# achinastone/Tensorium

Measured on AMD Instinct MI355X. Metric: fp32 SGEMM GFLOP/s (M=N=K=4096) + YOLOv3 conv-fwd images/s, higher is better.
Workload: dtype fp32; 1 GPU; sgemm_nn_4096x4096x4096; M=4096, N=4096, K=4096, parallelism=1 independent replicas, one process per GPU, no data-path collective

## Files before the change

tensorium_amd/csrc/conv1x1.hip:

```cpp
#include <algorithm>
#include <type_traits>

#include "tns_act.hpp"
#include "tns_internal.hpp"

namespace tns {
namespace {

typedef float floatx4 __attribute__((ext_vector_type(4)));

__device__ __forceinline__ void c1_dma16(const float* sbase, unsigned voff, unsigned lds) {
  unsigned keep;
  asm volatile(
      "s_mov_b32 %0, m0\n\ts_mov_b32 m0, %3\n\ts_nop 0\n\t"
      "global_load_lds_dwordx4 %1, %2\n\ts_mov_b32 m0, %0"
      : "=&s"(keep)
      : "v"(voff), "s"(sbase), "s"(lds)
      : "memory");
}

struct C1Args {
  const float* A;
  const float* X;
  float* C;
  const float* bias;
  int M, N, K, P, tiles_m, act;
  bool fuse;
  bool add;
};

template <int BM_, int BK_, int WM_, int WN_>
struct C1G {
  static constexpr int BM = BM_, BK = BK_, WM = WM_, WN = WN_;
  static constexpr int BN = 64 * WN, NW = WM * WN, NT = 64 * NW, NG = BK / 16;
  static constexpr int A_TILE = BK * BM, B_TILE = BK * BN, STAGE = A_TILE + B_TILE;
  static constexpr int AU = BM * BK / 4 / NT;
  static constexpr int RPI = 256 / BN;
  static constexpr int BDMA = BK / RPI;
  static constexpr int DPW = (BDMA + NW - 1) / NW;
  static_assert(BM == 16 * WM && BK % 16 == 0 && 256 % BN == 0 && BK % RPI == 0, "geometry");
  static_assert(AU >= 1 && BM * BK / 4 % NT == 0, "A units");
  static_assert(2 * STAGE * 4 <= 65536, "LDS: several blocks per CU");
  static_assert(NG % 2 == 0, "groups: f0 holds group 0 at every tile start");
};

template <int N>
__device__ __forceinline__ void c1_wait(bool keep_n) {
  if (keep_n)
    asm volatile("s_waitcnt vmcnt(%0)" ::"n"(N) : "memory");
  else
    asm volatile("s_waitcnt vmcnt(0)" ::: "memory");
}

template <class G>
__global__ __launch_bounds__(G::NT) void conv1x1_kernel(C1Args p) {
  constexpr int BM = G::BM, BN = G::BN, BK = G::BK, NG = G::NG;
  constexpr int A_TILE = G::A_TILE, STAGE = G::STAGE, AU = G::AU, DPW = G::DPW;
  __shared__ __attribute__((aligned(16))) float smem[2 * STAGE];
  const int tid = threadIdx.x, lane = tid & 63;
  const int w = __builtin_amdgcn_readfirstlane(tid >> 6), wm = w % G::WM, wn = w / G::WM;
  const int r16 = lane & 15, q = lane >> 4;
  int tm, tn;
  {
    const int nb = gridDim.x, bid = blockIdx.x;
    const int xcd = bid & 7, qq = nb >> 3, rr = nb & 7;
    const int wg = (xcd < rr ? xcd * (qq + 1) : rr * (qq + 1) + (xcd - rr) * qq) + (bid >> 3);
    tm = wg % p.tiles_m;
    tn = wg / p.tiles_m;
  }
  const int m0 = tm * BM, n0 = tn * BN;
  const int N = p.N, K = p.K, P = p.P, nt = K / BK;
  const unsigned lds0 = (unsigned)(uintptr_t)(__attribute__((address_space(3))) float*)smem;
  unsigned b_off;
  {
    int n = n0 + 4 * (lane % (BN / 4));
    if (n > N - 4) n = N - 4;
    const int img = n / P, pix = n - img * P;
    b_off = 4u * (unsigned)(img * K * P + (lane / (BN / 4)) * P + pix);
  }
  auto dma_b = [&](int t, int st, int v) {
    int u = w + G::NW * v;
    if (G::BDMA % G::NW != 0 && u >= G::BDMA) u -= G::NW;
    c1_dma16(p.X + (int64_t)(t * BK + u * G::RPI) * P, b_off,
             lds0 + 4u * (unsigned)(st * STAGE + A_TILE) + 1024u * (unsigned)u);
  };
  auto dma_all = [&](int t, int st) {
#pragma unroll
    for (int v = 0; v < DPW; ++v) dma_b(t, st, v);
  };
  unsigned a_off[AU];
  int a_dst[AU];
#pragma unroll
  for (int u = 0; u < AU; ++u) {
    const int idx = tid + G::NT * u;
    const int lo = idx & 7, rest = idx >> 3;
    const int m = rest % BM, kq4 = lo + 8 * (rest / BM);
    const int mr = m0 + m < p.M ? m : p.M - 1 - m0;
    a_off[u] = 4u * (unsigned)(mr * K + 4 * kq4);
    a_dst[u] = (4 * (kq4 >> 2)) * BM * 4 + m * 4 + (kq4 & 3);
  }
  const float* a_row0 = p.A + (int64_t)m0 * K;
  floatx4 ra[AU];
  auto load_a = [&](int t) {
    const float* sb = a_row0 + t * BK;
#pragma unroll
    for (int u = 0; u < AU; ++u)
      asm volatile("global_load_dwordx4 %0, %1, %2" : "=v"(ra[u]) : "v"(a_off[u]), "s"(sb) : "memory");
  };
  auto store_a = [&](int st) {
    float* as = smem + st * STAGE;
#pragma unroll
    for (int u = 0; u < AU; ++u) {
      asm volatile("" : "+v"(ra[u]));
      as[a_dst[u]] = ra[u][0];
      as[a_dst[u] + BM * 4] = ra[u][1];
      as[a_dst[u] + 2 * BM * 4] = ra[u][2];
      as[a_dst[u] + 3 * BM * 4] = ra[u][3];
    }
  };

  floatx4 acc[4];
#pragma unroll
  for (int j = 0; j < 4; ++j) acc[j] = floatx4{0.f, 0.f, 0.f, 0.f};
  struct Frag {
    floatx4 a, b[4];
  };
  auto frag = [&](int st, int g, Frag& f) {
    const float* ap = smem + st * STAGE + ((4 * g + q) * BM + wm * 16 + r16) * 4;
    f.a = *reinterpret_cast<const floatx4*>(ap);
    const float* bp = smem + st * STAGE + A_TILE + (16 * g + q) * BN + wn * 64 + 4 * r16;
#pragma unroll
    for (int i = 0; i < 4; ++i) f.b[i] = *reinterpret_cast<const floatx4*>(bp + 4 * i * BN);
  };
  auto mma = [&](const Frag& f) {
#pragma unroll
    for (int i = 0; i < 4; ++i)
#pragma unroll
      for (int j = 0; j < 4; ++j)
        acc[j] = __builtin_amdgcn_mfma_f32_16x16x4f32(f.a[i], f.b[i][j], acc[j], 0, 0, 0);
  };
  auto mma_dma = [&](const Frag& f, int tb, int st) {
    constexpr int NM = 16, STEP = NM / DPW > 0 ? NM / DPW : 1;
#pragma unroll
    for (int x = 0; x < NM; ++x) {
      const int i = x / 4, j = x % 4;
      acc[j] = __builtin_amdgcn_mfma_f32_16x16x4f32(f.a[i], f.b[i][j], acc[j], 0, 0, 0);
      if (x % STEP == 0 && x / STEP < DPW) dma_b(tb, st, x / STEP);
      __builtin_amdgcn_sched_barrier(0);
    }
    if constexpr (NM / STEP < DPW) {
#pragma unroll
      for (int v = NM / STEP; v < DPW; ++v) dma_b(tb, st, v);
    }
  };

  Frag f0, f1;
  load_a(0);
  dma_all(0, 0);
  c1_wait<0>(false);
  store_a(0);
  if (nt > 1) {
    load_a(1);
    dma_all(1, 1);
  }
  __syncthreads();
  frag(0, 0, f0);
  for (int t = 0; t < nt; ++t) {
    const int cur = t & 1, nxt = cur ^ 1;
#pragma unroll
    for (int g = 0; g + 1 < NG; ++g) {
      Frag& fc = (g & 1) ? f1 : f0;
      Frag& fn = (g & 1) ? f0 : f1;
      frag(cur, g + 1, fn);
      __builtin_amdgcn_sched_barrier(0);
      mma(fc);
      __builtin_amdgcn_sched_barrier(0);
    }
    Frag& fl = f1;
    Frag& ff = f0;
    if (t + 1 < nt) {
      c1_wait<0>(false);
      store_a(nxt);
      __syncthreads();
      frag(nxt, 0, ff);
      if (t + 2 < nt) {
        load_a(t + 2);
        __builtin_amdgcn_sched_barrier(0);
        mma_dma(fl, t + 2, cur);
      } else {
        __builtin_amdgcn_sched_barrier(0);
        mma(fl);
      }
    } else {
      mma(fl);
    }
  }

  const int n = n0 + wn * 64 + 4 * r16;
  if (n >= N) return;
  const int img = n / P, pix = n - img * P;
#pragma unroll
  for (int e = 0; e < 4; ++e) {
    const int m = m0 + wm * 16 + 4 * q + e;
    if (m >= p.M) continue;
    const float bi = p.fuse ? p.bias[m] : 0.0f;
    floatx4 v = {acc[0][e], acc[1][e], acc[2][e], acc[3][e]};
    if (p.fuse) {
#pragma unroll
      for (int j = 0; j < 4; ++j) v[j] = act_apply_cheap(v[j] + bi, p.act);
    }
    floatx4* cp = reinterpret_cast<floatx4*>(p.C + ((int64_t)img * p.M + m) * P + pix);
    if (p.add) {
      const floatx4 o = *cp;
#pragma unroll
      for (int j = 0; j < 4; ++j) v[j] = o[j] + v[j];
    }
    *cp = v;
  }
}

struct C1Form {
  int bm, bn, bk;
  hipError_t (*fn)(const C1Args&, hipStream_t);
  const char* name;
};

template <class G>
hipError_t launch_c1(const C1Args& a, hipStream_t s) {
  const int64_t blocks = (int64_t)a.tiles_m * ((a.N + G::BN - 1) / G::BN);
  hipLaunchKernelGGL((conv1x1_kernel<G>), dim3((unsigned)blocks), dim3(G::NT), 0, s, a);
  return hipGetLastError();
}

#define TNS_C1(BMv, BKv, WMv, WNv) \
  {BMv, 64 * WNv, BKv, launch_c1<C1G<BMv, BKv, WMv, WNv>>, "conv1x1<" #BMv "x" #WNv "x64x" #BKv ">"}
const C1Form kC1[] = {
    TNS_C1(32, 32, 2, 1),
    TNS_C1(64, 32, 4, 1),
    TNS_C1(32, 64, 2, 1),
    TNS_C1(32, 32, 2, 2),
    TNS_C1(16, 32, 1, 2),
};
#undef TNS_C1
constexpr int kNumC1 = sizeof(kC1) / sizeof(kC1[0]);

}

int conv1x1_count() { return kNumC1; }
const char* conv1x1_name(int v) { return v >= 0 && v < kNumC1 ? kC1[v].name : ""; }

int conv1x1_pick(int64_t M, int64_t N, int64_t K, int64_t P) {
  (void)M; (void)N;
  if (P % 4 || P < 2704 || K % 32) return -1;
  return 3;
}

__global__ __launch_bounds__(256) void c1_transpose_kernel(const float* __restrict__ in,
                                                           float* __restrict__ out, int rows,
                                                           int cols) {
  __shared__ float t[32][33];
  const int c0 = blockIdx.x * 32, r0 = blockIdx.y * 32;
  const int tx = threadIdx.x & 31, ty = threadIdx.x >> 5;
  for (int y = ty; y < 32; y += 8) {
    const int r = r0 + y, c = c0 + tx;
    t[y][tx] = r < rows && c < cols ? in[(int64_t)r * cols + c] : 0.0f;
  }
  __syncthreads();
  for (int y = ty; y < 32; y += 8) {
    const int c = c0 + y, r = r0 + tx;
    if (c < cols && r < rows) out[(int64_t)c * rows + r] = t[tx][y];
  }
}

hipError_t launch_transpose(const float* in, float* out, int64_t rows, int64_t cols,
                            hipStream_t s) {
  if (rows <= 0 || cols <= 0) return hipSuccess;
  if (rows > (1 << 26) || cols > (1 << 26)) return hipErrorInvalidValue;
  hipLaunchKernelGGL(c1_transpose_kernel,
                     dim3((unsigned)((cols + 31) / 32), (unsigned)((rows + 31) / 32)), dim3(256), 0,
                     s, in, out, (int)rows, (int)cols);
  return hipGetLastError();
}

hipError_t launch_conv1x1(int v, const float* weights, const float* x, const float* bias,
                          float* out, int64_t batch, int64_t M, int64_t K, int64_t P, int act,
                          hipStream_t s, bool add) {
  if (v < 0 || v >= kNumC1) return hipErrorInvalidValue;
  const C1Form& f = kC1[v];
  const int64_t N = batch * P;
  if (P % 4 || K % f.bk || M < 1 || N < 4 || batch * K * P * 4 > 0x7fffffffLL ||
      M * K * 4 > 0x7fffffffLL || (reinterpret_cast<uintptr_t>(weights) & 15) ||
      (reinterpret_cast<uintptr_t>(x) & 15) || (reinterpret_cast<uintptr_t>(out) & 15))
    return hipErrorInvalidValue;
  C1Args a{};
  a.A = weights; a.X = x; a.C = out; a.bias = bias;
  a.M = (int)M; a.N = (int)N; a.K = (int)K; a.P = (int)P;
  a.tiles_m = (int)((M + f.bm - 1) / f.bm); a.act = act; a.fuse = bias != nullptr; a.add = add;
  if ((int64_t)a.tiles_m * ((N + f.bn - 1) / f.bn) > 0x7fffffffLL) return hipErrorInvalidValue;
  return f.fn(a, s);
}

}
```

tensorium_amd/csrc/conv_slab.hip:

```cpp
#include <algorithm>
#include <type_traits>

#include "tns_act.hpp"
#include "tns_internal.hpp"

namespace tns {
namespace {

typedef float floatx4 __attribute__((ext_vector_type(4)));

__device__ __forceinline__ void slab_dma16(const float* sbase, unsigned voff, unsigned lds) {
  unsigned keep;
  asm volatile(
      "s_mov_b32 %0, m0\n\ts_mov_b32 m0, %3\n\ts_nop 0\n\t"
      "global_load_lds_dwordx4 %1, %2\n\ts_mov_b32 m0, %0"
      : "=&s"(keep)
      : "v"(voff), "s"(sbase), "s"(lds)
      : "memory");
}

struct SlabFillArgs {
  const float* x;
  int64_t strideX;
  float* slab;
  int C, H, W, stride, pad, dil, ow, ohw, N, K, KT;
  float inv_ohw, inv_ow;
  unsigned bytes;
  int64_t units;
};

__device__ __forceinline__ int slab_div(int n, int d, float inv) {
  int qq = (int)((float)n * inv);
  while (qq * d > n) --qq;
  while ((qq + 1) * d <= n) ++qq;
  return qq;
}

template <int KS, int BK, int BN>
__global__ __launch_bounds__(256) void slab_fill_kernel(SlabFillArgs a) {
  constexpr int NG = BK / 16, KK = KS * KS;
  const int64_t x = (int64_t)blockIdx.x * 256 + threadIdx.x;
  if (x >= a.units) return;
  const int c = (int)(x % BN);
  const int64_t r1 = x / BN;
  const int g = (int)(r1 % NG);
  const int64_t r2 = r1 / NG;
  const int t = (int)(r2 % a.KT), ct = (int)(r2 / a.KT);
  const int n = ct * BN + c;
  float v[16];
  const __amdgpu_buffer_rsrc_t rsrc =
      __builtin_amdgcn_make_buffer_rsrc(const_cast<float*>(a.x), 0, a.bytes, 0x00020000);
  {
    const int nn = n < a.N ? n : a.N - 1;
    const int img = slab_div(nn, a.ohw, a.inv_ohw), pix = nn - img * a.ohw;
    const int oy = slab_div(pix, a.ow, a.inv_ow), ox = pix - oy * a.ow;
    const int iy0 = oy * a.stride - a.pad, ix0 = ox * a.stride - a.pad;
    const int HW = a.H * a.W;
    unsigned mask = 0;
    int toff[KK];
#pragma unroll
    for (int kr = 0; kr < KS; ++kr)
#pragma unroll
      for (int kc = 0; kc < KS; ++kc) {
        const int iy = iy0 + kr * a.dil, ix = ix0 + kc * a.dil;
        mask |= (unsigned)(((unsigned)iy < (unsigned)a.H) & ((unsigned)ix < (unsigned)a.W))
                << (kr * KS + kc);
        toff[kr * KS + kc] = 4 * (kr * a.dil * a.W + kc * a.dil);
      }
    if (n >= a.N) mask = 0;
    const unsigned base = 4u * (unsigned)(img * (int)a.strideX + iy0 * a.W + ix0);
    const int k0 = t * BK + 16 * g;
    int ch = k0 / KK, tap = k0 - ch * KK;
#pragma unroll
    for (int e = 0; e < 16; ++e) {
      int off = toff[0];
#pragma unroll
      for (int u = 1; u < KK; ++u) off = tap == u ? toff[u] : off;
      const unsigned o = ((mask >> tap) & 1u) ? base + 4u * (unsigned)(ch * HW) + (unsigned)off
                                              : 0x80000000u;
      v[e] = __builtin_bit_cast(float, __builtin_amdgcn_raw_buffer_load_b32(rsrc, o, 0, 0));
      if (++tap == KK) {
        tap = 0;
        ++ch;
      }
    }
  }
  float* dst = a.slab + ((r2 * NG + g) * 4 * BN + c) * 4;
#pragma unroll
  for (int q = 0; q < 4; ++q)
    *reinterpret_cast<floatx4*>(dst + q * BN * 4) = floatx4{v[q], v[4 + q], v[8 + q], v[12 + q]};
}

template <int KS, int BK, int BN>
__global__ __launch_bounds__((BN + 63) / 64 * 64) void slab_fill_u_kernel(SlabFillArgs a) {
  constexpr int NG = BK / 16, KK = KS * KS;
  const int c = threadIdx.x;
  if (c >= BN) return;
  const int64_t r1 = blockIdx.x;
  const int g = (int)(r1 % NG);
  const int64_t r2 = r1 / NG;
  const int t = (int)(r2 % a.KT), ct = (int)(r2 / a.KT);
  const int n = ct * BN + c;
  float v[16];
  const __amdgpu_buffer_rsrc_t rsrc =
      __builtin_amdgcn_make_buffer_rsrc(const_cast<float*>(a.x), 0, a.bytes, 0x00020000);
  {
    const int nn = n < a.N ? n : a.N - 1;
    const int img = slab_div(nn, a.ohw, a.inv_ohw), pix = nn - img * a.ohw;
    const int oy = slab_div(pix, a.ow, a.inv_ow), ox = pix - oy * a.ow;
    const int iy0 = oy * a.stride - a.pad, ix0 = ox * a.stride - a.pad;
    const int HW = a.H * a.W;
    unsigned mask = 0;
#pragma unroll
    for (int kr = 0; kr < KS; ++kr)
#pragma unroll
      for (int kc = 0; kc < KS; ++kc) {
        const int iy = iy0 + kr * a.dil, ix = ix0 + kc * a.dil;
        mask |= (unsigned)(((unsigned)iy < (unsigned)a.H) & ((unsigned)ix < (unsigned)a.W))
                << (kr * KS + kc);
      }
    if (n >= a.N) mask = 0;
    const unsigned base = 4u * (unsigned)(img * (int)a.strideX + iy0 * a.W + ix0);
    const int k0 = __builtin_amdgcn_readfirstlane(t * BK + 16 * g);
    int ch = k0 / KK, tap = k0 - ch * KK;
    int kr = tap / KS, kc = tap - kr * KS;
#pragma unroll
    for (int e = 0; e < 16; ++e) {
      const unsigned uoff = 4u * (unsigned)(ch * HW + kr * a.dil * a.W + kc * a.dil);
      const unsigned o = ((mask >> tap) & 1u) ? base + uoff : 0x80000000u;
      v[e] = __builtin_bit_cast(float, __builtin_amdgcn_raw_buffer_load_b32(rsrc, o, 0, 0));
      ++tap;
      if (++kc == KS) {
        kc = 0;
        ++kr;
      }
      if (tap == KK) {
        tap = 0;
        kr = 0;
        ++ch;
      }
    }
  }
  float* dst = a.slab + ((r2 * NG + g) * 4 * BN + c) * 4;
#pragma unroll
  for (int q = 0; q < 4; ++q)
    *reinterpret_cast<floatx4*>(dst + q * BN * 4) = floatx4{v[q], v[4 + q], v[8 + q], v[12 + q]};
}

struct SlabGemmArgs {
  const float* A;
  const float* slab;
  float* C;
  const float* bias;
  int M, N, K, KT, tiles_m, ohw, act;
  bool fuse;
};

template <int BM_, int BN_, int BK_, int WM_, int WN_, int JA_, int NA_, int NS_, int DG_ = 0,
          int MAP_ = 0>
struct SG {
  static constexpr int BM = BM_, BN = BN_, BK = BK_, WM = WM_, WN = WN_, JA = JA_, NA = NA_;
  static constexpr int NS = NS_;
  static constexpr int DG = DG_, MAP = MAP_;
  static constexpr int NW = WM * WN, NT = 64 * NW, J = BN / 16, NG = BK / 16, ROWS = BK / 4;
  static constexpr int JB = NA < WN ? (J - NA * JA) / (WN - NA) : 0;
  static constexpr int A_TILE = ROWS * BM * 4, B_TILE = ROWS * BN * 4, STAGE = A_TILE + B_TILE;
  static constexpr int AU = BM * BK / 4 / NT;
  static constexpr int BDMA = 4 * BK * BN / 1024;
  static constexpr int DPW = (BDMA + NW - 1) / NW;
  static_assert(BM == 16 * WM && BN % 16 == 0 && BK % 16 == 0, "geometry");
  static_assert(NA * JA + (WN - NA) * JB == J && NA >= 1 && NA <= WN, "wave column split");
  static_assert(AU >= 1 && BM * BK / 4 % NT == 0, "A units");
  static_assert(4 * BK * BN % 1024 == 0, "whole DMA instructions");
  static_assert(NS >= 2 && NS * STAGE * 4 <= 163840, "LDS");
  static_assert(NG >= 2 && NG % 2 == 0, "groups: f0 holds group 0 at every tile start");
  static_assert(DPW * (NS - 2) <= 63 && DPW <= 63, "vmcnt immediates");
};

template <int JW>
struct SFrag {
  floatx4 a, b[JW];
};

template <int N>
__device__ __forceinline__ void wait_vm(bool keep_n) {
  if (keep_n)
    asm volatile("s_waitcnt vmcnt(%0)" ::"n"(N) : "memory");
  else
    asm volatile("s_waitcnt vmcnt(0)" ::: "memory");
}

template <class G>
__global__ __launch_bounds__(G::NT, 1) void slab_gemm_kernel(SlabGemmArgs p) {
  constexpr int BM = G::BM, BN = G::BN, BK = G::BK, NG = G::NG, NS = G::NS;
  constexpr int A_TILE = G::A_TILE, STAGE = G::STAGE, AU = G::AU, DPW = G::DPW;
  __shared__ __attribute__((aligned(16))) float smem[NS * STAGE];
  const int tid = threadIdx.x, lane = tid & 63;
  const int w = __builtin_amdgcn_readfirstlane(tid >> 6), wm = w % G::WM, wn = w / G::WM;
  const int r16 = lane & 15, q = lane >> 4;
  int tm, tn;
  {
    const int nb = gridDim.x, bid = blockIdx.x;
    const int xcd = bid & 7, qq = nb >> 3, rr = nb & 7;
    const int wg = (xcd < rr ? xcd * (qq + 1) : rr * (qq + 1) + (xcd - rr) * qq) + (bid >> 3);
    if constexpr (G::MAP == 1) {
      const int tiles_n = (p.N + BN - 1) / BN;
      tn = wg % tiles_n;
      tm = wg / tiles_n;
    } else {
      tm = wg % p.tiles_m;
      tn = wg / p.tiles_m;
    }
  }
  const int m0 = tm * BM, n0 = tn * BN;
  const int N = p.N, K = p.K, nt = p.KT;
  const float* slabT = p.slab + (int64_t)tn * K * BN;
  const unsigned lds0 = (unsigned)(uintptr_t)(__attribute__((address_space(3))) float*)smem;
  const unsigned voff = 16u * (unsigned)lane;
  auto dma_b = [&](int t, int st, int v) {
    if constexpr (G::DG & 1) return;
    int u = w + G::NW * v;
    if (G::BDMA % G::NW != 0 && u >= G::BDMA) u -= G::NW;
    slab_dma16(slabT + (int64_t)t * (BK * BN) + 256 * u, voff,
               lds0 + 4u * (unsigned)(st * STAGE + A_TILE) + 1024u * (unsigned)u);
  };
  auto dma_all = [&](int t, int st) {
#pragma unroll
    for (int v = 0; v < DPW; ++v) dma_b(t, st, v);
  };
  unsigned a_off[AU];
  int a_dst[AU];
#pragma unroll
  for (int u = 0; u < AU; ++u) {
    const int idx = tid + G::NT * u;
    const int lo = idx & 7, rest = idx >> 3;
    const int m = rest % BM, kq4 = lo + 8 * (rest / BM);
    a_off[u] = 4u * (unsigned)(m * K + 4 * kq4);
    a_dst[u] = (4 * (kq4 >> 2)) * BM * 4 + m * 4 + (kq4 & 3);
  }
  const float* a_row0 = p.A + (int64_t)m0 * K;
  floatx4 ra[AU];
  auto load_a = [&](int t) {
    if constexpr (G::DG & 2) return;
    const float* sb = a_row0 + t * BK;
#pragma unroll
    for (int u = 0; u < AU; ++u)
      asm volatile("global_load_dwordx4 %0, %1, %2" : "=v"(ra[u]) : "v"(a_off[u]), "s"(sb) : "memory");
  };
  auto store_a = [&](int st) {
    if constexpr (G::DG & 2) return;
    float* as = smem + st * STAGE;
#pragma unroll
    for (int u = 0; u < AU; ++u) {
      asm volatile("" : "+v"(ra[u]));
      as[a_dst[u]] = ra[u][0];
      as[a_dst[u] + BM * 4] = ra[u][1];
      as[a_dst[u] + 2 * BM * 4] = ra[u][2];
      as[a_dst[u] + 3 * BM * 4] = ra[u][3];
    }
  };

  auto run = [&](auto JWC, const int coff) {
    constexpr int JW = decltype(JWC)::value;
    floatx4 acc[JW];
#pragma unroll
    for (int j = 0; j < JW; ++j) acc[j] = floatx4{0.f, 0.f, 0.f, 0.f};
    using Frag = SFrag<JW>;
    auto frag = [&](int st, int g, Frag& f) {
      const float* ap = smem + st * STAGE + ((4 * g + q) * BM + wm * 16 + r16) * 4;
      f.a = *reinterpret_cast<const floatx4*>(ap);
      const float* bp = smem + st * STAGE + A_TILE + ((4 * g + q) * BN + coff * 16 + r16) * 4;
#pragma unroll
      for (int j = 0; j < JW; ++j) f.b[j] = *reinterpret_cast<const floatx4*>(bp + 64 * j);
    };
    auto mma = [&](const Frag& f) {
#pragma unroll
      for (int i = 0; i < 4; ++i)
#pragma unroll
        for (int j = 0; j < JW; ++j)
          acc[j] = __builtin_amdgcn_mfma_f32_16x16x4f32(f.a[i], f.b[j][i], acc[j], 0, 0, 0);
    };
    auto mma_dma = [&](const Frag& f, int tb, int st) {
      constexpr int NM = 4 * JW, STEP = NM / DPW > 0 ? NM / DPW : 1;
#pragma unroll
      for (int x = 0; x < NM; ++x) {
        const int i = x / JW, j = x % JW;
        acc[j] = __builtin_amdgcn_mfma_f32_16x16x4f32(f.a[i], f.b[j][i], acc[j], 0, 0, 0);
        if (x % STEP == 0 && x / STEP < DPW) dma_b(tb, st, x / STEP);
        __builtin_amdgcn_sched_barrier(0);
      }
      if constexpr (NM / STEP < DPW) {
#pragma unroll
        for (int v = NM / STEP; v < DPW; ++v) dma_b(tb, st, v);
      }
    };

    Frag f0, f1;
    load_a(0);
#pragma unroll
// ... 190 lines not shown
```

tensorium_amd/csrc/conv_tile4.hip:

```cpp
#include <type_traits>

#include "tns_act.hpp"
#include "tns_internal.hpp"

namespace tns {
namespace {

typedef float floatx4 __attribute__((ext_vector_type(4)));

template <int I, int N, class F>
__device__ __forceinline__ void cfor(F&& f) {
  if constexpr (I < N) {
    f(std::integral_constant<int, I>{});
    cfor<I + 1, N>(f);
  }
}

template <int JW>
struct Frag4 {
  floatx4 a, b[JW];
};

template <int BM_, int BN_, int WM_, int WN_, int BK_, int SG_, int IL_ = 0, bool SI_ = false,
          int RI_ = 0, bool ST_ = false, int JA_ = 0, int NA_ = 0, bool TA_ = false,
          bool DX_ = false, bool PF_ = false>
struct Geo4 {
  static constexpr bool PF = PF_;
  static constexpr bool DX = DX_;
  static constexpr bool TA = TA_;
  static constexpr int BM = BM_, BN = BN_, WM = WM_, WN = WN_, BK = BK_, SG = SG_;
  static constexpr int IL = IL_, RI = RI_;
  static constexpr bool SI = SI_, ST = ST_;
  static constexpr int NW = WM * WN, NT = 64 * NW;
  static constexpr int J = BN / 16;
  static constexpr int JA = JA_ > 0 ? JA_ : J / WN;
  static constexpr int NA = JA_ > 0 ? NA_ : WN;
  static constexpr int JB = NA < WN ? (J - NA * JA) / (WN - NA) : 0;
  static constexpr int NG = BK / 16;
  static constexpr int ROWS = BK / 4;
  static constexpr int A_TILE = ROWS * BM * 4;
  static constexpr int STAGE = ROWS * (BM + BN) * 4;
  static constexpr int AU = BM * BK / 4 / NT;
  static constexpr int KI = BK / 4 / NW;
  static_assert(BM == 16 * WM, "one 16-row strip per wave");
  static_assert(BM % 16 == 0 && BN % 16 == 0, "b128 slot rows: 64-dword multiples");
  static_assert(BK % 16 == 0 && SG <= NG - 2, "stores precede the barrier");
  static_assert(!(IL && SI) || SG >= 1 || PF_, "interleaved stores need a group after the loads");
  static_assert(!ST || (!IL && !SI && SG + 1 <= NG - 2 && NW % 2 == 0), "staggered staging");
  static_assert(AU >= 1 && BM * BK / 4 % NT == 0 && KI >= 1 && BK / 4 % NW == 0, "geometry");
  static_assert(NA * JA + (WN - NA) * JB == J && NA >= 1 && NA <= WN, "wave column split");
  static_assert(2 * STAGE * 4 + 64 <= 163840, "LDS");
  static_assert(!DX || TA, "DX: k-major weights");
  static_assert(!PF || !ST, "PF: register staging, no staggered halves");
  static constexpr int AST = 4 * AU;
  static constexpr int BLD = KI * J;
  static constexpr int BST = KI * J;
};

template <class G, int KS>
__global__ __launch_bounds__(G::NT) void conv_tile4_kernel(GemmArgs p, int dil) {
  constexpr int BM = G::BM, BN = G::BN, BK = G::BK, J = G::J, NG = G::NG;
  constexpr int A_TILE = G::A_TILE, STAGE = G::STAGE, AU = G::AU, KI = G::KI;
  __shared__ __attribute__((aligned(16))) float smem[2 * STAGE];
#ifdef TNS_CT4_STAMPS
  const unsigned long long rt_entry = __builtin_amdgcn_s_memrealtime();
#endif
  auto a_st = [&](int st) -> float* { return smem + st * STAGE; };
  auto b_st = [&](int st) -> float* { return smem + st * STAGE + A_TILE; };

  const int tid = threadIdx.x, lane = tid & 63, w = tid >> 6, wm = w % G::WM, wn = w / G::WM;
  const int half = __builtin_amdgcn_readfirstlane(w >= G::NW / 2 ? 1 : 0);
  const int r16 = lane & 15, q = lane >> 4;
  const int tiles_m = (int)(p.M / BM);
  int tm, tn;
  {
    const int nb = gridDim.x, bid = blockIdx.x;
    const int xcd = bid & 7, qq = nb >> 3, rr = nb & 7;
    const int wg = (xcd < rr ? xcd * (qq + 1) : rr * (qq + 1) + (xcd - rr) * qq) + (bid >> 3);
#if defined(TNS_CT4_MAP) && TNS_CT4_MAP == 1
    const int tiles_n = (int)((p.N + BN - 1) / BN);
    tn = wg % tiles_n;
    tm = wg / tiles_n;
#elif defined(TNS_CT4_MAP) && TNS_CT4_MAP == 2
    const int tiles_n = (int)((p.N + BN - 1) / BN);
    const int gm = min(4, tiles_m), per = gm * tiles_n, grp = wg / per;
    const int gs = min(gm, tiles_m - grp * gm), in = wg - grp * per;
    tm = grp * gm + in % gs;
    tn = in / gs;
#else
    tm = wg % tiles_m;
    tn = wg / tiles_m;
#endif
  }
  const int64_t m0 = (int64_t)tm * BM;
  const int n0 = tn * BN;
  const int N = (int)p.N, K = (int)p.K;
  const int H = p.conv_H, W = p.conv_W, HW = H * W;
  auto dx_pix = [&](int pix) -> int {
    if (!p.dx_cls) return pix;
    const int qy = pix / p.conv_ow, qx = pix - qy * p.conv_ow;
    return (2 * qy + ((p.dx_cls >> 1) & 1)) * p.dx_imgW + 2 * qx + ((p.dx_cls >> 2) & 1);
  };

  auto col_geo = [&](int n, unsigned& vb, unsigned& m) {
    n = n < N ? n : N - 1;
    const int img = n / p.conv_ohw, pix = n - img * p.conv_ohw;
    const int orow = pix / p.conv_ow, ocol = pix - orow * p.conv_ow;
    const int ir0 = orow * p.conv_sY - p.conv_pH, ic0 = ocol * p.conv_sX - p.conv_pW;
    vb = 4u * (unsigned)(img * (int)p.strideB + ir0 * W + ic0);
    m = 0;
#pragma unroll
    for (int kr = 0; kr < KS; ++kr)
#pragma unroll
      for (int kc = 0; kc < KS; ++kc)
        m |= (unsigned)(((unsigned)(ir0 + kr * dil) < (unsigned)H) &
                        ((unsigned)(ic0 + kc * dil) < (unsigned)W))
             << (kr * KS + kc);
  };
  unsigned vbase[J], tmask[J];
#pragma unroll
  for (int j = 0; j < J; ++j) col_geo(n0 + (16 * j + r16), vbase[j], tmask[j]);
  const __amdgpu_buffer_rsrc_t rsrc =
      __builtin_amdgcn_make_buffer_rsrc(const_cast<float*>(p.B), 0, p.conv_bytes, 0x00020000);

  int kc_[KI], kr_[KI], cc_[KI];
#pragma unroll
  for (int ii = 0; ii < KI; ++ii) {
    const int sl = w * KI + ii;
    const int k = 16 * (sl >> 2) + 4 * q + (sl & 3);
    if constexpr (G::DX) {
      cc_[ii] = k;
      kr_[ii] = kc_[ii] = 0;
      continue;
    }
    cc_[ii] = k / (KS * KS);
    const int rem = k - cc_[ii] * KS * KS;
    kr_[ii] = rem / KS;
    kc_[ii] = rem - kr_[ii] * KS;
  }
  const int F_ = G::DX ? K / (p.dx_cls ? (p.dx_taps >> 16) : KS * KS) : 0;
  int d_f0 = 0, d_t = 0;
  auto advance = [&]() {
    if constexpr (G::DX) {
      d_f0 += BK;
      if (d_f0 == F_) {
        d_f0 = 0;
        ++d_t;
      }
      return;
    }
#pragma unroll
    for (int ii = 0; ii < KI; ++ii) {
      if constexpr (KS == 1) {
        cc_[ii] += BK;
      } else {
        constexpr int DC = BK / (KS * KS), DR = BK % (KS * KS);
        int rem = kr_[ii] * KS + kc_[ii] + DR;
        int c = cc_[ii] + DC;
        if (rem >= KS * KS) { rem -= KS * KS; ++c; }
        cc_[ii] = c;
        kr_[ii] = rem >= 2 * KS ? 2 : (rem >= KS ? 1 : 0);
        kc_[ii] = rem - kr_[ii] * KS;
      }
    }
  };
  using S0 = std::integral_constant<int, 0>;
  using S1 = std::integral_constant<int, 1>;
  float rbs[G::PF ? 2 : 1][KI][J];
  auto gather_b = [&](auto SET) {
    auto& rb = rbs[decltype(SET)::value];
#pragma unroll
    for (int ii = 0; ii < KI; ++ii) {
      int y = kr_[ii] * dil, z = kc_[ii] * dil, tap = kr_[ii] * KS + kc_[ii], cc = cc_[ii];
      if constexpr (G::DX) {
        int fr = KS - 1 - d_t / KS, fc = KS - 1 - d_t % KS;
        if (p.dx_cls) {
          const int fb = (p.dx_taps >> (4 * d_t)) & 15;
          fr = fb / KS;
          fc = fb - fr * KS;
        }
        y = fr;
        z = fc;
        tap = fr * KS + fc;
        cc = d_f0 + cc_[ii];
      }
      const unsigned x = 4u * (unsigned)(cc * HW + y * W + z);
#pragma unroll
      for (int j = 0; j < J; ++j) {
#if defined(TNS_CT4_DIAG) && (TNS_CT4_DIAG & 1)
        rb[ii][j] = (float)(x + j);
#else
        const bool ok = __builtin_amdgcn_ubfe(tmask[j], tap, 1) != 0;
        const unsigned off = ok ? vbase[j] + x : 0x80000000u;
        rb[ii][j] = __builtin_bit_cast(float, __builtin_amdgcn_raw_buffer_load_b32(rsrc, off, 0, 0));
#endif
      }
    }
  };
  int b_dst[KI];
#pragma unroll
  for (int ii = 0; ii < KI; ++ii) b_dst[ii] = (w * KI + ii) * BN * 4 + r16 * 4 + q;
  auto store_b = [&](float* bs, auto SET) {
    auto& rb = rbs[decltype(SET)::value];
#if defined(TNS_CT4_DIAG) && (TNS_CT4_DIAG & 2)
    return;
#endif
#pragma unroll
    for (int ii = 0; ii < KI; ++ii)
// ... 138 lines not shown
    constexpr bool more = decltype(MORE)::value;
    constexpr int par = decltype(PAR)::value;
    using SL = std::integral_constant<int, G::PF ? par : 0>;
    using SS = std::integral_constant<int, G::PF ? par ^ 1 : 0>;
    const int tc = t & 1, tx = (t + 1) & 1;
    TNS_PH(5);
    if constexpr (more && G::PF && !G::IL) {
      advance();
      load_a(min((t + 2) * BK, K - BK), SL{});
      gather_b(SL{});
      __builtin_amdgcn_sched_barrier(0);
    } else if constexpr (more && !G::IL && !G::ST && !G::PF) {
      advance();
      load_a((t + 1) * BK, S0{});
      gather_b(S0{});
      __builtin_amdgcn_sched_barrier(0);
    }
    TNS_PH(0);
#pragma unroll
    for (int g = 0; g < NG; ++g) {
      Frag& fc = (g & 1) ? f1 : f0;
      Frag& fn = (g & 1) ? f0 : f1;
      if constexpr (more)
        if (g == NG - 1) {
          TNS_PH(3);
#ifdef TNS_CT4_STAMPS
          if (t == 8 && lane == 0 && p.stamps != nullptr && blockIdx.x < (1u << 16) && w < 16)
            p.stamps[32 * blockIdx.x + 16 + w] =
                (unsigned)(__builtin_amdgcn_s_memtime() & 0xffffffffu);
#endif
          __syncthreads();
          TNS_PH(4);
        }
      __builtin_amdgcn_sched_barrier(0);
      if constexpr (more && G::ST)
        if (g < 2 && half == g) {
          advance();
          load_a((t + 1) * BK, S0{});
          gather_b(S0{});
          __builtin_amdgcn_sched_barrier(0);
        }
      const bool reads = g + 1 < NG || more;
      if (g + 1 < NG)
        frag(tc, g + 1, fn);
      else if (more)
        frag(tx, 0, fn);
      if constexpr (more && G::IL) {
        if (g == 0) {
          advance();
          if constexpr (G::PF) {
            load_a(min((t + 2) * BK, K - BK), SL{});
            gather_b(SL{});
          } else {
            load_a((t + 1) * BK, S0{});
            gather_b(S0{});
          }
        }
      }
      if constexpr (more && G::SI) {
        if (g == G::SG) {
          store_a(a_st(tx), SS{});
          store_b(b_st(tx), SS{});
        }
      }
      mma(fc);
      if constexpr (G::RI > 0 || G::IL > 0 || G::SI) {
#pragma unroll
        for (int i = 0; i < 4 * JW; ++i) {
          __builtin_amdgcn_sched_group_barrier(0x008, 1, 0);
          if constexpr (G::RI > 0)
            if (reads && i % G::RI == 0 && i / G::RI < JW + 1)
              __builtin_amdgcn_sched_group_barrier(0x100, 1, 0);
          if constexpr (more && G::IL > 0)
            if (g == 0) {
              __builtin_amdgcn_sched_group_barrier(0x002, G::IL, 0);
              if (i < AU + G::BLD) __builtin_amdgcn_sched_group_barrier(0x020, 1, 0);
            }
          if constexpr (more && G::SI)
            if (g == G::SG && i < G::AST + G::BST)
              __builtin_amdgcn_sched_group_barrier(0x200, 1, 0);
        }
      }
      __builtin_amdgcn_sched_barrier(0);
      if constexpr (more && G::ST)
        if (g >= G::SG && g <= G::SG + 1 && g == G::SG + half) {
          store_a(a_st(tx), S0{});
          store_b(b_st(tx), S0{});
          __builtin_amdgcn_sched_barrier(0);
        }
      if constexpr (more && !G::SI && !G::ST)
        if (g == G::SG) {
          TNS_PH(1);
          store_a(a_st(tx), SS{});
          store_b(b_st(tx), SS{});
          __builtin_amdgcn_sched_barrier(0);
          TNS_PH(2);
        }
    }
    if constexpr (G::DX) flush();
  };
  static_assert(NG % 2 == 0, "f0 holds group 0 at every tile start");
  if constexpr (G::PF) {
    int t = 0;
    for (; t + 2 < nt; t += 2) {
      tile(t, std::true_type{}, S0{});
      tile(t + 1, std::true_type{}, S1{});
    }
    if (t + 1 < nt) {
      tile(t, std::true_type{}, S0{});
      tile(t + 1, std::false_type{}, S1{});
    } else if (t < nt) {
      tile(t, std::false_type{}, S0{});
    }
  } else {
    for (int t = 0; t + 1 < nt; ++t) tile(t, std::true_type{}, S0{});
    if (nt > 0) tile(nt - 1, std::false_type{}, S0{});
  }

#ifdef TNS_CT4_STAMPS
  TNS_PH(5);
  if (tid == 0 && p.stamps != nullptr && blockIdx.x < (1u << 16)) {
    unsigned* st = p.stamps + 32 * blockIdx.x;
    for (int i = 0; i < 6; ++i) st[i] = (unsigned)ph[i];
    st[6] = (unsigned)(tl - tk0);
    const unsigned long long rt_loop = __builtin_amdgcn_s_memrealtime();
    st[7] = (unsigned)nt | (unsigned)(rt_loop - rt0) << 8;
    st[8] = (unsigned)rt_entry;
    st[9] = (unsigned)(rt_entry >> 32);
    st[10] = (unsigned)(rt0 - rt_entry);
    st[12] = (unsigned)(rt_loop - rt_entry);
  }
#endif
#undef TNS_PH
  const bool fuse = p.epi == EPI_BIAS_ACT;
  const int act = p.act;
  if constexpr (G::DX) {
    const int64_t row0 = m0 + wm * 16 + 4 * q;
#pragma unroll
    for (int j = 0; j < JW; ++j) {
      const int n = n0 + coff * 16 + 16 * j + r16;
      if (n >= N) continue;
      const int img = n / p.conv_ohw, pix = dx_pix(n - img * p.conv_ohw);
      float* cp = p.C + (int64_t)img * p.strideC + pix + row0 * p.ldc;
#pragma unroll
      for (int e = 0; e < 4; ++e) cp[e * p.ldc] = rs[j][e];
    }
    return;
  }
  const bool add = p.epi == EPI_ADD;
  const int64_t row0 = m0 + wm * 16 + 4 * q;
  float bias[4];
#pragma unroll
  for (int e = 0; e < 4; ++e) bias[e] = fuse ? p.bias[row0 + e] : 0.0f;
#pragma unroll
  for (int j = 0; j < JW; ++j) {
    const int n = n0 + coff * 16 + 16 * j + r16;
    if (n >= N) continue;
    const int img = n / p.conv_ohw, pix = n - img * p.conv_ohw;
    float* cp = p.C + (int64_t)img * p.strideC + pix + row0 * p.ldc;
#pragma unroll
    for (int e = 0; e < 4; ++e) {
      float v = acc[j][e];
      if (fuse) v = act_apply_cheap(v + bias[e], act);
      if (add) v = cp[e * p.ldc] + v;
      cp[e * p.ldc] = v;
    }
  }
#ifdef TNS_CT4_STAMPS
  if (tid == 0 && p.stamps != nullptr && blockIdx.x < (1u << 16)) {
    asm volatile("s_waitcnt vmcnt(0)" ::: "memory");
    p.stamps[32 * blockIdx.x + 11] = (unsigned)(__builtin_amdgcn_s_memrealtime() - rt_entry);
  }
#endif
  };
  if constexpr (G::NA == G::WN) {
    run(std::integral_constant<int, G::JA>{}, wn * G::JA);
  } else {
    if (__builtin_amdgcn_readfirstlane(wn) < G::NA)
      run(std::integral_constant<int, G::JA>{}, wn * G::JA);
    else
      run(std::integral_constant<int, G::JB>{}, G::NA * G::JA + (wn - G::NA) * G::JB);
  }
}

#ifdef TNS_CT4_STAMPS
unsigned* g_ct4_stamps = nullptr;
#endif

template <class G>
hipError_t launch_g4(const GemmArgs& a_in, int ks, int dil, hipStream_t s) {
  GemmArgs a = a_in;
#ifdef TNS_CT4_STAMPS
  a.stamps = g_ct4_stamps;
#endif
  if (a.M % G::BM || a.K % G::BK || a.K <= 0) return hipErrorInvalidValue;
  if (!G::TA && (a.lda % 4 || (reinterpret_cast<uintptr_t>(a.A) & 15))) return hipErrorInvalidValue;
  if (G::TA && (a.lda < a.M || a.K * a.lda > 0x7fffffffLL)) return hipErrorInvalidValue;
  const int64_t tiles = (a.M / G::BM) * ((a.N + G::BN - 1) / G::BN);
  if (tiles > 0x7fffffff || a.N > 0x7fffffff || a.K > 0x7fffffff) return hipErrorInvalidValue;
  if (ks == 3)
    hipLaunchKernelGGL((conv_tile4_kernel<G, 3>), dim3((unsigned)tiles), dim3(G::NT), 0, s, a, dil);
  else if (ks == 1)
    hipLaunchKernelGGL((conv_tile4_kernel<G, 1>), dim3((unsigned)tiles), dim3(G::NT), 0, s, a, dil);
  else
    return hipErrorInvalidValue;
  return hipGetLastError();
}

struct TileInfo4 {
  int bm, bn, bk;
  hipError_t (*fn)(const GemmArgs&, int, int, hipStream_t);
  const char* name;
};
#define TNS_CT4(BMv, BNv, WMv, WNv, BKv, SGv, ILv, SIv, RIv, STv)                      \
  {BMv, BNv, BKv, launch_g4<Geo4<BMv, BNv, WMv, WNv, BKv, SGv, ILv, SIv, RIv, STv>>,    \
   "conv_tile4<" #BMv "x" #BNv "x" #BKv ",w" #WMv "x" #WNv ",g" #SGv ",il" #ILv ",si" #SIv \
   ",ri" #RIv ",st" #STv ">"}
#define TNS_CT4U(BMv, BNv, WMv, WNv, BKv, SGv, SIv, RIv, JAv, NAv)                      \
  {BMv, BNv, BKv, launch_g4<Geo4<BMv, BNv, WMv, WNv, BKv, SGv, 0, SIv, RIv, false, JAv, NAv>>, \
   "conv_tile4<" #BMv "x" #BNv "x" #BKv ",w" #WMv "x" #WNv ",g" #SGv ",si" #SIv ",ri" #RIv    \
   ",j" #JAv "x" #NAv ">"}
#define TNS_CT4P(BMv, BNv, WMv, WNv, BKv, SGv, SIv, RIv, JAv, NAv)                           \
  {BMv, BNv, BKv,                                                                             \
   launch_g4<Geo4<BMv, BNv, WMv, WNv, BKv, SGv, 0, SIv, RIv, false, JAv, NAv, false, false,  \
                  true>>,                                                                    \
   "conv_tile4_pf<" #BMv "x" #BNv "x" #BKv ",w" #WMv "x" #WNv ",g" #SGv ",si" #SIv ",ri" #RIv \
   ",j" #JAv "x" #NAv ">"}
#define TNS_CT4PI(BMv, BNv, WMv, WNv, BKv, SGv, ILv, SIv, RIv, JAv, NAv)                     \
  {BMv, BNv, BKv,                                                                             \
   launch_g4<Geo4<BMv, BNv, WMv, WNv, BKv, SGv, ILv, SIv, RIv, false, JAv, NAv, false, false, \
                  true>>,                                                                    \
   "conv_tile4_pf<" #BMv "x" #BNv "x" #BKv ",w" #WMv "x" #WNv ",g" #SGv ",il" #ILv ",si" #SIv  \
   ",ri" #RIv ",j" #JAv "x" #NAv ">"}
const TileInfo4 kTiles4[] = {
    TNS_CT4(128, 176, 8, 1, 32, 0, 0, false, 0, false),
    TNS_CT4(128, 176, 8, 1, 64, 2, 0, false, 0, false),
    TNS_CT4(128, 176, 8, 1, 64, 1, 0, true, 3, false),
    TNS_CT4(128, 176, 8, 1, 64, 1, 0, true, 2, false),
    TNS_CT4(128, 176, 8, 1, 64, 1, 0, false, 3, true),
    TNS_CT4(128, 176, 8, 1, 64, 1, 0, false, 0, true),
    TNS_CT4(128, 176, 8, 1, 64, 1, 0, false, 2, true),
    TNS_CT4(64, 96, 4, 1, 32, 0, 0, false, 0, false),
    TNS_CT4(64, 96, 4, 1, 32, 0, 0, false, 3, false),
    TNS_CT4(64, 192, 4, 2, 64, 1, 0, false, 3, true),
    TNS_CT4(64, 96, 4, 2, 64, 1, 0, false, 3, true),
    TNS_CT4(64, 64, 4, 2, 32, 0, 0, false, 0, false),
    TNS_CT4(64, 64, 4, 1, 32, 0, 0, false, 0, false),
    TNS_CT4(64, 32, 4, 1, 32, 0, 0, false, 0, false),
    TNS_CT4(64, 32, 4, 2, 32, 0, 0, false, 0, false),
    TNS_CT4(64, 64, 4, 1, 64, 2, 0, false, 0, false),
    TNS_CT4(64, 32, 4, 1, 64, 2, 0, false, 0, false),
    TNS_CT4U(64, 176, 4, 2, 64, 1, true, 2, 6, 1),
    TNS_CT4U(64, 176, 4, 2, 32, 0, false, 3, 6, 1),
    TNS_CT4U(32, 176, 2, 4, 64, 1, true, 2, 3, 3),
    TNS_CT4(128, 48, 8, 1, 32, 0, 0, false, 3, false),
    TNS_CT4(128, 48, 8, 1, 64, 1, 0, true, 2, false),
    TNS_CT4(64, 48, 4, 1, 32, 0, 0, false, 3, false),
    TNS_CT4(64, 48, 4, 1, 64, 1, 0, true, 2, false),
    TNS_CT4(128, 96, 8, 1, 64, 1, 0, true, 2, false),
    TNS_CT4P(64, 32, 4, 1, 32, 0, false, 0, 0, 0),
    TNS_CT4PI(64, 176, 4, 2, 32, 0, 2, false, 3, 6, 1),
    TNS_CT4PI(64, 176, 4, 2, 32, 0, 0, true, 3, 6, 1),
};
#define TNS_CT4T(BMv, BNv, WMv, WNv, BKv, SGv, SIv, RIv, JAv, NAv)                      \
  {BMv, BNv, BKv,                                                                      \
   launch_g4<Geo4<BMv, BNv, WMv, WNv, BKv, SGv, 0, SIv, RIv, false, JAv, NAv, true>>,  \
   "conv_tile4_ta<" #BMv "x" #BNv "x" #BKv ",w" #WMv "x" #WNv ",g" #SGv ",si" #SIv     \
   ",ri" #RIv ",j" #JAv "x" #NAv ">"}
#define TNS_CT4TP(BMv, BNv, WMv, WNv, BKv, SGv, SIv, RIv, JAv, NAv)                      \
  {BMv, BNv, BKv,                                                                      \
   launch_g4<Geo4<BMv, BNv, WMv, WNv, BKv, SGv, 0, SIv, RIv, false, JAv, NAv, true, false, \
                  true>>,                                                               \
   "conv_tile4_ta_pf<" #BMv "x" #BNv "x" #BKv ",w" #WMv "x" #WNv ",g" #SGv ",si" #SIv   \
   ",ri" #RIv ",j" #JAv "x" #NAv ">"}
const TileInfo4 kTiles4T[] = {
    TNS_CT4T(128, 176, 8, 1, 64, 1, true, 2, 0, 0),
    TNS_CT4T(128, 96, 8, 1, 64, 1, true, 2, 0, 0),
    TNS_CT4T(128, 48, 8, 1, 64, 1, true, 2, 0, 0),
    TNS_CT4T(64, 176, 4, 2, 32, 0, false, 3, 6, 1),
    TNS_CT4T(64, 96, 4, 1, 32, 0, false, 3, 0, 0),
    TNS_CT4T(64, 32, 4, 1, 32, 0, false, 0, 0, 0),
    TNS_CT4T(128, 176, 8, 1, 32, 0, false, 3, 0, 0),
    TNS_CT4T(64, 64, 4, 2, 32, 0, false, 3, 0, 0),
    TNS_CT4T(64, 64, 4, 1, 32, 0, false, 3, 0, 0),
    TNS_CT4T(128, 64, 8, 1, 32, 0, false, 3, 0, 0),
    TNS_CT4T(64, 128, 4, 2, 32, 0, false, 3, 0, 0),
    TNS_CT4TP(64, 96, 4, 1, 32, 0, false, 3, 0, 0),
    TNS_CT4TP(64, 64, 4, 2, 32, 0, false, 3, 0, 0),
    TNS_CT4TP(128, 48, 8, 1, 64, 1, true, 2, 0, 0),
};
constexpr int kNumTiles4T = sizeof(kTiles4T) / sizeof(kTiles4T[0]);
#define TNS_CT4DX(BMv, BNv, WMv, WNv, BKv, SGv, SIv, RIv, JAv, NAv)                          \
  {BMv, BNv, BKv,                                                                          \
   launch_g4<Geo4<BMv, BNv, WMv, WNv, BKv, SGv, 0, SIv, RIv, false, JAv, NAv, true, true>>, \
   "conv_tile4_dx<" #BMv "x" #BNv "x" #BKv ",w" #WMv "x" #WNv ",g" #SGv ",si" #SIv         \
   ",ri" #RIv ",j" #JAv "x" #NAv ">"}
#define TNS_CT4DXP(BMv, BNv, WMv, WNv, BKv, SGv, SIv, RIv, JAv, NAv)                         \
  {BMv, BNv, BKv,                                                                          \
   launch_g4<Geo4<BMv, BNv, WMv, WNv, BKv, SGv, 0, SIv, RIv, false, JAv, NAv, true, true,   \
                  true>>,                                                                  \
   "conv_tile4_dx_pf<" #BMv "x" #BNv "x" #BKv ",w" #WMv "x" #WNv ",g" #SGv ",si" #SIv      \
   ",ri" #RIv ",j" #JAv "x" #NAv ">"}
const TileInfo4 kTiles4DX[] = {
    TNS_CT4DX(64, 176, 4, 2, 32, 0, false, 3, 6, 1),
    TNS_CT4DX(64, 96, 4, 1, 32, 0, false, 3, 0, 0),
    TNS_CT4DX(64, 48, 4, 1, 32, 0, false, 3, 0, 0),
    TNS_CT4DX(128, 96, 8, 1, 64, 1, true, 2, 0, 0),
    TNS_CT4DX(64, 64, 4, 2, 32, 0, false, 3, 0, 0),
    TNS_CT4DX(128, 48, 8, 1, 64, 1, true, 2, 0, 0),
    TNS_CT4DX(32, 176, 2, 4, 64, 1, true, 2, 3, 3),
    TNS_CT4DXP(64, 176, 4, 2, 32, 0, false, 3, 6, 1),
    TNS_CT4DXP(64, 64, 4, 2, 32, 0, false, 3, 0, 0),
    TNS_CT4DXP(32, 176, 2, 4, 64, 1, true, 2, 3, 3),
    TNS_CT4DXP(64, 48, 4, 1, 32, 0, false, 3, 0, 0),
};
constexpr int kNumTiles4DX = sizeof(kTiles4DX) / sizeof(kTiles4DX[0]);
#undef TNS_CT4DX
#undef TNS_CT4DXP
// ... 198 lines not shown
```

Before: 148,600 GFLOP/s.

## Stage conv tile epilogue through LDS for 16-byte row stores with write-through policy

Adds a store16 helper offering plain, nontemporal and sc1 write-through stores, plus a row-staging epilogue. For selected conv_tile4 tile shapes the wave transposes its accumulators through LDS so each lane writes contiguous 16-byte row segments instead of scattered scalar column stores. By default it uses the sc1 store policy and reuses pipeline stage buffers, sometimes in halves or after a block barrier. This trades extra LDS traffic and wave barriers for coalesced, wider global writes. The conv1x1 and slab-fill paths get the hook but default to plain stores.

```diff
diff --git a/tensorium_amd/csrc/conv1x1.hip b/tensorium_amd/csrc/conv1x1.hip
--- a/tensorium_amd/csrc/conv1x1.hip
+++ b/tensorium_amd/csrc/conv1x1.hip
@@ -1,8 +1,13 @@
 #include <algorithm>
 #include <type_traits>
 
+#include "conv_store16.hpp"
 #include "tns_act.hpp"
 #include "tns_internal.hpp"
+
+#ifndef TNS_C1_STORE
+#define TNS_C1_STORE 0
+#endif
 
 namespace tns {
 namespace {
@@ -209,13 +214,15 @@
 #pragma unroll
       for (int j = 0; j < 4; ++j) v[j] = act_apply_cheap(v[j] + bi, p.act);
     }
-    floatx4* cp = reinterpret_cast<floatx4*>(p.C + ((int64_t)img * p.M + m) * P + pix);
+    float* cp = p.C + ((int64_t)img * p.M + m) * P + pix;
     if (p.add) {
-      const floatx4 o = *cp;
+      const floatx4 o = *reinterpret_cast<const floatx4*>(cp);
 #pragma unroll
       for (int j = 0; j < 4; ++j) v[j] = o[j] + v[j];
-    }
-    *cp = v;
+      *reinterpret_cast<floatx4*>(cp) = v;
+    } else {
+      store16<TNS_C1_STORE>(cp, v);
+    }
   }
 }
 
diff --git a/tensorium_amd/csrc/conv_slab.hip b/tensorium_amd/csrc/conv_slab.hip
--- a/tensorium_amd/csrc/conv_slab.hip
+++ b/tensorium_amd/csrc/conv_slab.hip
@@ -1,8 +1,13 @@
 #include <algorithm>
 #include <type_traits>
 
+#include "conv_store16.hpp"
 #include "tns_act.hpp"
 #include "tns_internal.hpp"
+
+#ifndef TNS_SLAB_FILL_STORE
+#define TNS_SLAB_FILL_STORE 0
+#endif
 
 namespace tns {
 namespace {
@@ -88,7 +93,7 @@
   float* dst = a.slab + ((r2 * NG + g) * 4 * BN + c) * 4;
 #pragma unroll
   for (int q = 0; q < 4; ++q)
-    *reinterpret_cast<floatx4*>(dst + q * BN * 4) = floatx4{v[q], v[4 + q], v[8 + q], v[12 + q]};
+    store16<TNS_SLAB_FILL_STORE>(dst + q * BN * 4, floatx4{v[q], v[4 + q], v[8 + q], v[12 + q]});
 }
 
 template <int KS, int BK, int BN>
@@ -144,7 +149,7 @@
   float* dst = a.slab + ((r2 * NG + g) * 4 * BN + c) * 4;
 #pragma unroll
   for (int q = 0; q < 4; ++q)
-    *reinterpret_cast<floatx4*>(dst + q * BN * 4) = floatx4{v[q], v[4 + q], v[8 + q], v[12 + q]};
+    store16<TNS_SLAB_FILL_STORE>(dst + q * BN * 4, floatx4{v[q], v[4 + q], v[8 + q], v[12 + q]});
 }
 
 struct SlabGemmArgs {
diff --git a/tensorium_amd/csrc/conv_store16.hpp b/tensorium_amd/csrc/conv_store16.hpp
--- /dev/null
+++ b/tensorium_amd/csrc/conv_store16.hpp
@@ -0,0 +1,62 @@
+#pragma once
+
+#include <hip/hip_runtime.h>
+
+#include <cstdint>
+
+namespace tns {
+
+typedef float st16_f4 __attribute__((ext_vector_type(4)));
+
+enum { ST16_PLAIN = 0, ST16_NT = 1, ST16_WT = 2 };
+
+template <int POLICY>
+__device__ __forceinline__ void store16(float* p, st16_f4 v) {
+  static_assert(POLICY >= ST16_PLAIN && POLICY <= ST16_WT, "store policy");
+  if constexpr (POLICY == ST16_WT) {
+    asm volatile("global_store_dwordx4 %0, %1, off sc1\n\ts_nop 1" ::"v"(p), "v"(v) : "memory");
+  } else if constexpr (POLICY == ST16_NT) {
+    __builtin_nontemporal_store(v, reinterpret_cast<st16_f4*>(p));
+  } else {
+    *reinterpret_cast<st16_f4*>(p) = v;
+  }
+}
+
+template <int JW>
+struct RowStage {
+  static constexpr int RS = 16 * JW + 4;
+  static constexpr int FLOATS = 16 * RS;
+};
+
+__device__ __forceinline__ bool rows_store16_ok(const float* C, int64_t strideC, int64_t ldc,
+                                                int ohw) {
+  return ((ohw | (int)ldc | (int)strideC) & 3) == 0 && (reinterpret_cast<uintptr_t>(C) & 15) == 0;
+}
+
+template <int JW, int POLICY>
+__device__ __forceinline__ void rows_store16(float* stage, const st16_f4* v, int lane,
+                                             float* C, int64_t strideC, int64_t ldc, int64_t row0,
+                                             int col0, int N, int ohw) {
+  constexpr int RS = RowStage<JW>::RS, GW = 4 * JW;
+  const int r16 = lane & 15, q = lane >> 4;
+  asm volatile("" ::: "memory");
+#pragma unroll
+  for (int j = 0; j < JW; ++j)
+#pragma unroll
+    for (int e = 0; e < 4; ++e) stage[(4 * q + e) * RS + 16 * j + r16] = v[j][e];
+  __builtin_amdgcn_fence(__ATOMIC_RELEASE, "workgroup");
+  __builtin_amdgcn_wave_barrier();
+  __builtin_amdgcn_fence(__ATOMIC_ACQUIRE, "workgroup");
+#pragma unroll
+  for (int i = 0; i < JW; ++i) {
+    const int idx = 64 * i + lane;
+    const int r = idx / GW, g = idx - r * GW;
+    const st16_f4 x = *reinterpret_cast<const st16_f4*>(stage + r * RS + 4 * g);
+    const int n = col0 + 4 * g;
+    if (n >= N) continue;
+    const int img = n / ohw, pix = n - img * ohw;
+    store16<POLICY>(C + (int64_t)img * strideC + (row0 + r) * ldc + pix, x);
+  }
+}
+
+}
diff --git a/tensorium_amd/csrc/conv_tile4.hip b/tensorium_amd/csrc/conv_tile4.hip
--- a/tensorium_amd/csrc/conv_tile4.hip
+++ b/tensorium_amd/csrc/conv_tile4.hip
@@ -1,7 +1,18 @@
 #include <type_traits>
 
+#include "conv_store16.hpp"
 #include "tns_act.hpp"
 #include "tns_internal.hpp"
+
+#ifndef TNS_CT4_ROWSTORE
+#define TNS_CT4_ROWSTORE 7
+#endif
+#ifndef TNS_CT4_STORE
+#define TNS_CT4_STORE 2
+#endif
+#ifndef TNS_CT4_ROWSTORE_BARRIER
+#define TNS_CT4_ROWSTORE_BARRIER 0
+#endif
 
 namespace tns {
 namespace {
@@ -54,6 +65,16 @@
   static_assert(!PF || !ST, "PF: register staging, no staggered halves");
   static constexpr int AST = 4 * AU;
   static constexpr int BLD = KI * J;
+  static constexpr int RSW = RowStage<(JA > JB ? JA : JB)>::FLOATS;
+  static constexpr bool ROWSTORE =
+      !TA && !DX && BN % 4 == 0 && NW * RSW <= 2 * STAGE &&
+      (((TNS_CT4_ROWSTORE & 1) && BM == 128 && BN == 176) || ((TNS_CT4_ROWSTORE & 2) && BN == 96) ||
+       ((TNS_CT4_ROWSTORE & 4) && BN == 32));
+  static constexpr int JH = ((JA > JB ? JA : JB) + 1) / 2;
+  static constexpr int RSH = RowStage<JH>::FLOATS;
+  static constexpr bool ROWSTORE_HALVES =
+      !TNS_CT4_ROWSTORE_BARRIER && NW * RSW > STAGE && NW * RSH <= STAGE;
+  static constexpr bool ROWSTORE_FREE = !TNS_CT4_ROWSTORE_BARRIER && NW * RSW <= STAGE;
   static constexpr int BST = KI * J;
 };
 
@@ -498,18 +519,48 @@
   float bias[4];
 #pragma unroll
   for (int e = 0; e < 4; ++e) bias[e] = fuse ? p.bias[row0 + e] : 0.0f;
-#pragma unroll
-  for (int j = 0; j < JW; ++j) {
-    const int n = n0 + coff * 16 + 16 * j + r16;
-    if (n >= N) continue;
-    const int img = n / p.conv_ohw, pix = n - img * p.conv_ohw;
-    float* cp = p.C + (int64_t)img * p.strideC + pix + row0 * p.ldc;
-#pragma unroll
-    for (int e = 0; e < 4; ++e) {
-      float v = acc[j][e];
-      if (fuse) v = act_apply_cheap(v + bias[e], act);
-      if (add) v = cp[e * p.ldc] + v;
-      cp[e * p.ldc] = v;
+  bool stored = false;
+  if constexpr (G::ROWSTORE) {
+    if (!add && rows_store16_ok(p.C, p.strideC, p.ldc, p.conv_ohw)) {
+      if (fuse) {
+#pragma unroll
+        for (int j = 0; j < JW; ++j)
+#pragma unroll
+          for (int e = 0; e < 4; ++e) acc[j][e] = act_apply_cheap(acc[j][e] + bias[e], act);
+      }
+      if constexpr (G::ROWSTORE_FREE) {
+        rows_store16<JW, TNS_CT4_STORE>(smem + (nt & 1) * STAGE + w * G::RSW, acc, lane, p.C,
+                                        p.strideC, p.ldc, m0 + wm * 16, n0 + coff * 16, N,
+                                        p.conv_ohw);
+      } else if constexpr (G::ROWSTORE_HALVES) {
+        constexpr int J0 = (JW + 1) / 2;
+        float* stage = smem + (nt & 1) * STAGE + w * G::RSH;
+        rows_store16<J0, TNS_CT4_STORE>(stage, acc, lane, p.C, p.strideC, p.ldc, m0 + wm * 16,
+                                        n0 + coff * 16, N, p.conv_ohw);
+        rows_store16<JW - J0, TNS_CT4_STORE>(stage, acc + J0, lane, p.C, p.strideC, p.ldc,
+                                             m0 + wm * 16, n0 + (coff + J0) * 16, N, p.conv_ohw);
+      } else {
+        __syncthreads();
+        rows_store16<JW, TNS_CT4_STORE>(smem + w * G::RSW, acc, lane, p.C, p.strideC, p.ldc,
+                                        m0 + wm * 16, n0 + coff * 16, N, p.conv_ohw);
+      }
+      stored = true;
+    }
+  }
+  if (!stored) {
+#pragma unroll
+    for (int j = 0; j < JW; ++j) {
+      const int n = n0 + coff * 16 + 16 * j + r16;
+      if (n >= N) continue;
+      const int img = n / p.conv_ohw, pix = n - img * p.conv_ohw;
+      float* cp = p.C + (int64_t)img * p.strideC + pix + row0 * p.ldc;
+#pragma unroll
+      for (int e = 0; e < 4; ++e) {
+        float v = acc[j][e];
+        if (fuse) v = act_apply_cheap(v + bias[e], act);
+        if (add) v = cp[e * p.ldc] + v;
+        cp[e * p.ldc] = v;
+      }
     }
   }
 #ifdef TNS_CT4_STAMPS
```

Result: no change. 148,800 GFLOP/s (median of 4 runs) (+0.1%).
